# Asunatan/LM-Net

Measured on AMD Instinct MI355X. Metric: train images/sec at 352x352, 1/2/4/8 MI355X; Dice vs ref, higher is better.
Workload: dtype f32; 1 GPU; LM-Net fp32 training step (fwd + CE/Dice loss + bwd + AdamW), batch 8/GPU, 352x352 synthetic disc masks (BASELINE configs[1]); global_batch=8, parallelism=dp1, launch=lmn_plan_run (recorded C-side schedule, one crossing per pass)

## Files before the change

lm_net_amd/csrc/conv_common.h:

```cpp
#pragma once
#include "common.h"
#include <stdlib.h>

struct ConvParams {
  lmn_conv_args_t a;
  int nkb[3];
  int kb_off[3];
  int NKB;
  int NCTT;
  int ncls;
  int gpi;
  int ng_c[4];
  int Hc[4], Wc[4];
  int total_sets;
  float inv_keep_ep;
  float inv_keep_src[3];
  int TH, TW, TP, NG, XH, XW, CS, CKB, tiles_x, tiles_y, total_tiles;
  uint32_t mTW, mXW;
  int strided;
  float* det_stats;
  LmnLay lay_src[3], lay_out, lay_aux;
  int32_t rpw;
  uint32_t rp_magic;
  LmnLay lay_out2, lay_aux2;
  int32_t NCTT2;
  int32_t prio;
};

__device__ __forceinline__ void lmn_wave_prio(int mode) {
  uint32_t slot;
  asm volatile("s_getreg_b32 %0, hwreg(HW_REG_HW_ID, 0, 4)" : "=s"(slot));
  const uint32_t p = mode >= 4 ? (uint32_t)(7 - mode) : (mode == 2 ? 3u - (slot & 3u) : (mode == 3 ? (slot & 1u) * 3u : (slot & 3u)));
  switch (p) {
    case 0: __builtin_amdgcn_s_setprio(0); break;
    case 1: __builtin_amdgcn_s_setprio(1); break;
    case 2: __builtin_amdgcn_s_setprio(2); break;
    default: __builtin_amdgcn_s_setprio(3); break;
  }
}

__device__ __forceinline__ void lmn_wave_stagger(int units) {
  uint32_t slot;
  asm volatile("s_getreg_b32 %0, hwreg(HW_REG_HW_ID, 0, 4)" : "=s"(slot));
  const int n = (int)(slot & 7u) * units;
  for (int i = 0; i < n; ++i) __builtin_amdgcn_s_sleep(4);
}

namespace {

template <int PM> struct ActT { typedef float type; };
template <> struct ActT<2> { typedef lmn_bf16 type; };

typedef short s16x4 __attribute__((ext_vector_type(4)));
typedef __bf16 bf16x2_t __attribute__((ext_vector_type(2)));
typedef float f32x2_t __attribute__((ext_vector_type(2)));
__device__ __forceinline__ uint32_t pk_bf16(float a, float b) {
  const f32x2_t t = {a, b};
  return __builtin_bit_cast(uint32_t, __builtin_convertvector(t, bf16x2_t));
}
__device__ __forceinline__ uint2 pk4_bf16(f32x4 v) { return uint2{pk_bf16(v[0], v[1]), pk_bf16(v[2], v[3])}; }
template <bool BF> struct Frag { typedef f32x4 type; };
template <> struct Frag<true> { typedef uint2 type; };
template <bool BF> __device__ __forceinline__ typename Frag<BF>::type ldfrag(const float* p) {
  if constexpr (BF) return *reinterpret_cast<const uint2*>(p);
  else return *reinterpret_cast<const f32x4*>(p);
}
__device__ __forceinline__ f32x4 mfma_bf16(uint2 a, uint2 b, f32x4 c) {
  return __builtin_amdgcn_mfma_f32_16x16x16bf16_1k(__builtin_bit_cast(s16x4, a), __builtin_bit_cast(s16x4, b), c, 0, 0, 0);
}
typedef __bf16 bf16x8_t __attribute__((ext_vector_type(8)));
__device__ __forceinline__ f32x4 mfma_bf16x2(uint2 a0, uint2 a1, uint2 b0, uint2 b1, f32x4 c) {
#ifdef LMN_MFMA_X2
  const uint4 a = uint4{a0.x, a0.y, a1.x, a1.y}, b = uint4{b0.x, b0.y, b1.x, b1.y};
  return __builtin_amdgcn_mfma_f32_16x16x32_bf16(__builtin_bit_cast(bf16x8_t, a), __builtin_bit_cast(bf16x8_t, b), c, 0, 0, 0);
#else
  return mfma_bf16(a1, b1, mfma_bf16(a0, b0, c));
#endif
}

#ifdef LMN_CT_TIMING
__device__ unsigned long long g_ct_timing[4096 * 8];
#define LMN_TK(i) do { tk_b = __builtin_amdgcn_s_memtime(); tk_s[i] += tk_b - tk_a; tk_a = tk_b; } while (0)
#define LMN_TK_DRAIN() __builtin_amdgcn_s_waitcnt(0)
#else
#define LMN_TK(i) do { } while (0)
#define LMN_TK_DRAIN() do { } while (0)
#endif

}

int lmn_launch_conv_tile_1x1(const ConvParams& T, dim3 grid, size_t shmem, hipStream_t st, int tnct, int pm, int ek, bool rp, bool ln);
int lmn_launch_conv_tile_3x3(const ConvParams& T, dim3 grid, size_t shmem, hipStream_t st, int tnct, int pm, int ek, bool wlk, bool up);
int lmn_launch_conv_tile_3x3g(const ConvParams& T, dim3 grid, size_t shmem, hipStream_t st, int tnct, int pm, int ek, bool wlk);
size_t lmn_conv_dma3_lds(int C, int nct);
int lmn_launch_conv_dma3(const ConvParams& T, int blocks, hipStream_t st);
size_t lmn_conv_dmaM_lds(int XH, int XW);
bool lmn_conv_dmaM_fits(int XH, int XW);
int lmn_launch_conv_dmaM(const ConvParams& T, dim3 grid, hipStream_t st, int ek);
int lmn_conv_dma1_tp(int ks0, int ks1, int ks2, int aq, int nct, int mode, int gs, int nct2, int mode2);
size_t lmn_conv_dma1_lds(int ks0, int ks1, int ks2, int aq, int nct, int tp, int nct2);
int lmn_launch_conv_dma1(const ConvParams& T, int ks0, int ks1, int ks2, int aq, int nct, int mode, int gs, int nct2, int mode2, int blocks, hipStream_t st);
int lmn_launch_conv_tile_s2t(const ConvParams& T, dim3 grid, size_t shmem, hipStream_t st, int tnct, int pm, int ek);
int lmn_launch_conv_tileM(const ConvParams& T, dim3 grid, size_t shmem, hipStream_t st, int taps, int ncw, int pm, int ek, bool rp, bool ln, bool up);
```

lm_net_amd/csrc/conv_fwd.hip:

```cpp
#include "conv_common.h"

namespace {

struct PackGeom {
  int taps, Cout, Cin, nsrc, cs[3], transposed, row_off, rows;
  int bf16;
};

__device__ __forceinline__ float pack_element(const float* __restrict__ w, const PackGeom& g, int64_t i) {
  int nkb[3], kboff[3], cbase[3], NKB = 0, cb = 0;
#pragma unroll
  for (int s = 0; s < 3; ++s) {
    nkb[s] = s < g.nsrc ? (g.cs[s] + 15) / 16 : 0;
    kboff[s] = NKB;
    cbase[s] = cb;
    NKB += nkb[s];
    cb += s < g.nsrc ? g.cs[s] : 0;
  }
  const int nrows = g.transposed ? g.rows : g.Cout;
  const int NCTT = (nrows + 15) / 16;
  const int j = (int)(i & 3);
  const int lane = (int)((i >> 2) & 63);
  uint32_t t = (uint32_t)(i >> 8);
  const int ct = (int)(t % (uint32_t)NCTT);
// ... 148 lines not shown
  if (c < cinw) {
    const float zx = be[e] * m[c] + acc;
    dW[(int64_t)e * cinw + c] += a * R[(int64_t)e * rows + c] + b * zx + k * m[c];
  } else if (db) {
    const float zs = count * be[e] + acc;
    db[e] += a * hstats[e] + b * zs + k * count;
  }
}

}

thread_local char g_lmn_err[256] = {0};

extern "C" {

int lmn_abi_version(void) { return LMN_ABI_VERSION; }
int lmn_sizeof_conv_args(void) { return (int)sizeof(lmn_conv_args_t); }
int lmn_sizeof_src(void) { return (int)sizeof(lmn_src_t); }
int lmn_sizeof_pack_job(void) { return (int)sizeof(lmn_pack_job_t); }
const char* lmn_last_error(void) { return g_lmn_err; }
#ifdef LMN_CT_TIMING
int lmn_ct_timing(unsigned long long* out, int n) {
  return (int)hipMemcpyFromSymbol(out, HIP_SYMBOL(g_ct_timing), sizeof(unsigned long long) * n);
}
#endif

int64_t lmn_conv_pack_size(int ksize, int Cout, int nsrc, const int32_t* c) {
  int64_t nkb = 0;
  for (int s = 0; s < nsrc; ++s) nkb += (c[s] + 15) / 16;
  return (int64_t)ksize * ksize * nkb * ((Cout + 15) / 16) * 256;
}

int lmn_conv_pack(const float* w, float* wpack, int ksize, int Cout, int Cin, int nsrc, const int32_t* c,
                  int transposed, int row_off, int rows, int dtype, lmn_stream_t stream) {
  LMN_REQUIRE(w && wpack && c, "conv_pack: null pointer");
  LMN_REQUIRE(dtype == LMN_F32 || dtype == LMN_BF16, "conv_pack: dtype %d", dtype);
  if (g_lmn_rec && nsrc >= 1 && nsrc <= 3) {
    int32_t cc[3] = {c[0], nsrc > 1 ? c[1] : 0, nsrc > 2 ? c[2] : 0};
    const int32_t c0 = cc[0], c1 = cc[1], c2 = cc[2];
    lmn_rec_push([=]() -> int { const int32_t ca[3] = {c0, c1, c2}; return lmn_conv_pack(w, wpack, ksize, Cout, Cin, nsrc, ca, transposed, row_off, rows, dtype, stream); }, "lmn_conv_pack(");
  }
  LMN_REQUIRE(ksize == 1 || ksize == 3, "conv_pack: ksize %d", ksize);
  LMN_REQUIRE(nsrc >= 1 && nsrc <= 3, "conv_pack: nsrc %d", nsrc);
  int csum = 0;
  for (int s = 0; s < nsrc; ++s) csum += c[s];
  if (!transposed) {
    LMN_REQUIRE(csum == Cin || (nsrc == 1 && csum > Cin && csum < Cin + 4),
                "conv_pack: sources sum to %d channels, weight has %d", csum, Cin);
  } else {
    LMN_REQUIRE(nsrc == 1 && c[0] >= Cout && c[0] < Cout + 4, "conv_pack(transposed): one source of Cout=%d channels expected", Cout);
    LMN_REQUIRE(row_off >= 0 && rows > 0 && row_off + rows < Cin + 4, "conv_pack(transposed): rows [%d,+%d) of %d", row_off, rows, Cin);
  }
  const int nrows = transposed ? rows : (Cout + 3) / 4 * 4;
  const int64_t total = lmn_conv_pack_size(ksize, nrows, nsrc, c);
  LMN_REQUIRE(total < (1LL << 31), "conv_pack: %lld packed elements (32-bit index arithmetic)", (long long)total);
  const int blocks = (int)((total + 255) / 256 > 4096 ? 4096 : (total + 255) / 256);
  PackGeom g;
  g.taps = ksize * ksize; g.Cout = Cout; g.Cin = Cin; g.nsrc = nsrc;
  g.cs[0] = c[0]; g.cs[1] = nsrc > 1 ? c[1] : 0; g.cs[2] = nsrc > 2 ? c[2] : 0;
  g.transposed = transposed; g.row_off = row_off; g.rows = rows;
  g.bf16 = dtype == LMN_BF16;
  LMN_LAUNCH(conv_pack_kernel, dim3(blocks), dim3(256), 0, (hipStream_t)stream, w, wpack, g, total);
  return lmn_launch_status("conv_pack");
}

int lmn_conv_pack_batch(const lmn_pack_job_t* jobs_dev, int njobs, int64_t total_blocks, lmn_stream_t stream) {
  LMN_REC(lmn_conv_pack_batch(jobs_dev, njobs, total_blocks, stream));
  LMN_REQUIRE(jobs_dev && njobs > 0 && total_blocks > 0 && total_blocks < (1LL << 31), "conv_pack_batch: bad job table");
  LMN_LAUNCH(conv_pack_batch_kernel, dim3((unsigned)total_blocks), dim3(256), 0, (hipStream_t)stream, jobs_dev, njobs);
  return lmn_launch_status("conv_pack_batch");
}

static int g_conv_dma_mode = -1;
static int g_conv_dma_min_tiles = 512;
int lmn_conv_dma_config(int mode, int min_tiles) {
  const int prev = g_conv_dma_mode;
  if (mode >= 0) g_conv_dma_mode = mode;
  if (min_tiles >= 0) g_conv_dma_min_tiles = min_tiles;
  return prev;
}

struct Dma1Sel { int ks[3]; int aq, nct, mode, gs, nct2, mode2, tp; };
static bool dma1_select(const lmn_conv_args_t& A, Dma1Sel& S) {
  if (g_conv_dma_mode < 0) { const char* e = getenv("LMN_CONV_DMA"); g_conv_dma_mode = e ? atoi(e) : 7; }
  if (!(g_conv_dma_mode & 2)) return false;
  if (A.ksize != 1 || A.stride != 1 || A.mma_dtype != LMN_F32 || A.act_dtype != LMN_F32 || A.drop_p != 0.f || A.fin.mode != LMN_FIN_NONE || A.residual) return false;
  if (A.nsrc < 1 || A.nsrc > 3 || A.Cout <= 0 || A.Cout % 4 || A.Cout > 48 || A.out_rp_w < 0) return false;
  if (A.Hin != A.Hout || A.Win != A.Wout) return false;
  S.ks[0] = S.ks[1] = S.ks[2] = 0;
  S.gs = 0;
  for (int s = 0; s < A.nsrc; ++s) {
    const lmn_src_t& X = A.src[s];
    if (!X.ptr || X.C <= 0 || X.C % 4 || X.C > 48) return false;
    if (s == 0 && X.flags == LMN_SRC_GELU) S.gs = 1;
    else if (X.flags != 0 || X.scale) return false;
    if (X.rp_w && X.rp_w != A.Win) return false;
    S.ks[s] = X.C / 4;
  }
  if ((A.out_rp_w && A.out_rp_w != A.Win) || (A.aux && A.aux_rp_w && A.aux_rp_w != A.Win)) return false;
  const bool sebwd = A.epilogue == LMN_EP_SE_BWD && A.stats_mode == LMN_STATS_EP && A.aux && A.stats;
  S.mode = sebwd ? 5 : ((A.epilogue == LMN_EP_LINEAR && A.stats_mode == LMN_STATS_SUM_SQ && A.stats) ? 2 : ((A.epilogue == LMN_EP_LINEAR && A.stats_mode == LMN_STATS_NONE) ? 0 : -1));
  if (S.mode < 0 || (!sebwd && A.aux)) return false;
  S.nct = (A.Cout + 15) / 16;
  S.aq = sebwd ? A.Cout / 4 : 0;
  S.nct2 = S.mode2 = 0;
  int64_t maxc = A.Cout > A.out_cstride ? A.Cout : A.out_cstride;
  if (sebwd && A.aux_cstride > maxc) maxc = A.aux_cstride;
  for (int s = 0; s < A.nsrc; ++s) maxc = A.src[s].cstride > maxc ? A.src[s].cstride : maxc;
  const lmn_conv_chain_t& C2 = A.chain;
  if (C2.wpack) {
    if (S.mode != 0 || !A.out || !C2.out || C2.Cout <= 0 || C2.Cout % 4 || C2.Cout > 48 || g_lmn_det) return false;
    if ((C2.out_rp_w && C2.out_rp_w != A.Win) || (C2.aux && C2.aux_rp_w && C2.aux_rp_w != A.Win)) return false;
    const bool se2 = C2.epilogue == LMN_EP_SE_BWD && C2.stats_mode == LMN_STATS_EP && C2.aux && C2.stats;
    const bool sq2 = C2.epilogue == LMN_EP_LINEAR && C2.stats_mode == LMN_STATS_SUM_SQ && C2.stats && !C2.aux && C2.stats_rep >= 1;
    if (!se2 && !sq2) return false;
    S.mode2 = se2 ? 5 : 2;
    S.nct2 = (C2.Cout + 15) / 16;
    S.aq = se2 ? C2.Cout / 4 : 0;
    if (C2.Cout > maxc) maxc = C2.Cout;
    if (C2.out_cstride > maxc) maxc = C2.out_cstride;
    if (se2 && C2.aux_cstride > maxc) maxc = C2.aux_cstride;
  }
  S.tp = lmn_conv_dma1_tp(S.ks[0], S.ks[1], S.ks[2], S.aq, S.nct, S.mode, S.gs, S.nct2, S.mode2);
  if (S.tp <= 0) return false;
  const int64_t hw = (int64_t)A.Hin * A.Win, npx = (int64_t)A.B * hw;
  return hw % S.tp == 0 && npx / S.tp >= g_conv_dma_min_tiles && npx * maxc * 4 < 0x7fffffffLL;
}

int lmn_conv_chain_ok(const lmn_conv_args_t* args) {
  if (!args || !args->chain.wpack) return 0;
  Dma1Sel S;
  return dma1_select(*args, S) ? 1 : 0;
}

int lmn_conv_fwd(const lmn_conv_args_t* args, lmn_stream_t stream) {
  LMN_REQUIRE(args, "conv_fwd: null args");
  if (g_lmn_rec) {
    const lmn_conv_args_t copy = *args;
    lmn_rec_push([copy, stream]() -> int { return lmn_conv_fwd(&copy, stream); }, "lmn_conv_fwd(");
  }
  const lmn_conv_args_t& A = *args;
  if (A.chain.wpack) {
    Dma1Sel Sc;
    LMN_REQUIRE(dma1_select(A, Sc), "conv_fwd: these arguments do not take a chained second conv (lmn_conv_chain_ok says so beforehand)");
  }
  LMN_REQUIRE(A.ksize == 1 || A.ksize == 3, "conv_fwd: ksize %d", A.ksize);
  LMN_REQUIRE(A.stride == 1 || A.stride == 2, "conv_fwd: stride %d", A.stride);
  LMN_REQUIRE(A.nsrc >= 1 && A.nsrc <= 3, "conv_fwd: nsrc %d", A.nsrc);
  LMN_REQUIRE(A.Cout > 0 && A.Cout % 4 == 0, "conv_fwd: Cout %d must be a positive multiple of 4", A.Cout);
  LMN_REQUIRE(A.mma_dtype == LMN_F32 || A.mma_dtype == LMN_BF16, "conv_fwd: mma_dtype %d", A.mma_dtype);
  LMN_REQUIRE(A.act_dtype == LMN_F32 || (A.act_dtype == LMN_BF16 && A.mma_dtype == LMN_BF16),
              "conv_fwd: act_dtype %d with mma_dtype %d (bf16 storage needs bf16 matrix-core operands)", A.act_dtype, A.mma_dtype);
  LMN_REQUIRE(A.B > 0 && A.Hout > 0 && A.Wout > 0 && A.Hin > 0 && A.Win > 0, "conv_fwd: empty tensor");
  LMN_REQUIRE(A.wpack, "conv_fwd: null packed weights");
  LMN_REQUIRE(A.out || A.stats, "conv_fwd: neither out nor stats requested");
  LMN_REQUIRE(!(A.transposed && A.nsrc != 1), "conv_fwd: transposed form takes one source");
  {
    static int trace = -1;
    if (trace < 0) { const char* e = getenv("LMN_CONV_TRACE"); trace = e ? atoi(e) : 0; }
    if (trace) {
      fprintf(stderr, "conv_fwd k%d s%d T%d B%d %dx%d->%dx%d nsrc%d C", A.ksize, A.stride, A.transposed, A.B, A.Hin, A.Win, A.Hout, A.Wout, A.nsrc);
      for (int s = 0; s < A.nsrc; ++s) fprintf(stderr, "%s%d/%d(f%d%s%s)", s ? "+" : "", A.src[s].C, A.src[s].cstride, A.src[s].flags, A.src[s].scale ? "s" : "", A.src[s].rp_w ? "r" : "");
      fprintf(stderr, " Cout%d/%d ep%d st%d act%d drop%g res%d aux%d fin%d mma%d adt%d orp%d bias%d%d\n", A.Cout, A.out_cstride, A.epilogue, A.stats_mode, A.act, (double)A.drop_p,
              A.residual != nullptr, A.aux != nullptr, A.fin.mode, A.mma_dtype, A.act_dtype, A.out_rp_w, A.bias != nullptr, A.bias2 != nullptr);
    }
  }
  ConvParams P;
// ... 234 lines not shown
    int maxkb = 0;
    for (int s = 0; s < a.nsrc; ++s) maxkb = P.nkb[s] > maxkb ? P.nkb[s] : maxkb;
    T.CKB = maxkb < 2 ? maxkb : 2;
    if (ncw && a.ksize == 1) {
      static int ckb_cap = -1;
      if (ckb_cap < 0) { const char* e = getenv("LMN_CONVM_CKB"); ckb_cap = e ? atoi(e) : 8; }
      int c = maxkb < ckb_cap ? maxkb : ckb_cap;
      while (c > 2 && (size_t)T.TP * (c * 16 + 8) * sizeof(float) > 37 * 1024) --c;
      if (c > T.CKB) T.CKB = c;
    }
    if (ncw && a.ksize == 3 && !up2) {
      static int ckb3_env = -1;
      if (ckb3_env < 0) { const char* e = getenv("LMN_CONVM_CKB3"); ckb3_env = e ? atoi(e) : 8; }
      const long mblk = (long)a.B * ((gW + T.TW - 1) / T.TW) * ((gH + T.TH - 1) / T.TH) * ((P.NCTT + 4 * ncw - 1) / (4 * ncw));
      const size_t lds_cap = mblk <= 288 ? 144 * 1024 : (mblk <= 576 ? 72 * 1024 : 0);
      for (int c = 8; c > 2; c >>= 1) {
        if (c > ckb3_env || c > maxkb) continue;
        const bool bf0 = a.mma_dtype == LMN_BF16;
        const size_t need = ((size_t)T.XH * T.XW * (c * (bf0 ? 8 : 16) + (bf0 ? 4 : 8)) + (2 + 9) * 4 * ncw * 16) * sizeof(float);
        if (need <= lds_cap) { T.CKB = c; break; }
      }
    }
    T.CS = T.CKB * 16 + (st_in == 1 ? 8 : 4);
    const bool bf = a.mma_dtype == LMN_BF16;
    const int pm = bf ? (a.act_dtype == LMN_BF16 ? 2 : 1) : 0;
    if (bf) T.CS = T.CKB * 8 + 4;
    T.tiles_x = (gW + T.TW - 1) / T.TW;
    T.tiles_y = (gH + T.TH - 1) / T.TH;
    T.total_tiles = a.B * T.tiles_x * T.tiles_y;
    T.strided = a.epilogue == LMN_EP_SE_BWD ? 0 : 1;
    T.mTW = (uint32_t)((1ull << 32) / (uint32_t)T.TW + 1);
    T.mXW = (uint32_t)((1ull << 32) / (uint32_t)T.XW + 1);
    LMN_REQUIRE(T.XH * T.XW < 65536, "conv_fwd: window too large");
    size_t shmem = ((size_t)T.XH * T.XW * T.CS + (2 + 9) * tnct * 16) * sizeof(float);
    static int wl_kb = -1;
    if (wl_kb < 0) { const char* e = getenv("LMN_CONV_WL_KB"); wl_kb = e ? atoi(e) : 32; }
    const size_t wl_bytes = (size_t)9 * T.CKB * tnct * (a.mma_dtype == LMN_BF16 ? 128 : 256) * sizeof(float);
    const bool wlk = a.ksize == 3 && !s2t && shmem + wl_bytes <= (size_t)wl_kb * 1024;
    if (wlk) shmem += wl_bytes;
    LMN_REQUIRE(ncw || shmem <= 64 * 1024, "conv_fwd: LDS window %zu B", shmem);
    int blocks = T.total_tiles;
    int maxb = 1280 / tchunks > 256 ? 1280 / tchunks : 256;
    if (npg == 4) {
      int per_cu = (int)((160 * 1024) / (shmem + 512));
      per_cu = per_cu > 5 ? 5 : (per_cu < 1 ? 1 : per_cu);
      maxb = 256 * per_cu / tchunks > 256 ? 256 * per_cu / tchunks : 256;
    }
    if (s2t) maxb = 320 / tchunks > 64 ? 320 / tchunks : 64;
    {
      static int maxb_env = -1;
      if (maxb_env < 0) { const char* e = getenv("LMN_CONV_MAXB"); maxb_env = e ? atoi(e) : 0; }
      if (maxb_env > 0 && a.ksize == 3 && !s2t) maxb = maxb_env / tchunks > 1 ? maxb_env / tchunks : 1;
    }
    if (blocks > maxb) blocks = maxb;
    int ek = 1;
    if (a.epilogue <= LMN_EP_AFFINE_ACT && a.stats_mode == LMN_STATS_NONE) ek = 0;
    else if (a.drop_p > 0.f) ek = 1;
    else if (a.epilogue == LMN_EP_LINEAR && a.stats_mode == LMN_STATS_SUM_SQ) ek = 2;
    else if (a.epilogue == LMN_EP_BN_BWD1 && a.stats_mode == LMN_STATS_EP) ek = 3;
    else if (a.epilogue == LMN_EP_BN_BWD2 && a.stats_mode == LMN_STATS_NONE) ek = 4;
    else if (a.epilogue == LMN_EP_SE_BWD && a.stats_mode == LMN_STATS_EP) ek = 5;
    else if (a.epilogue == LMN_EP_LN_BWD) ek = 6;
    int det_ns = 0;
    int64_t det_sz = 0;
    auto det_prep = [&](int nbx) -> int {
      if (!g_lmn_det || !a.stats || a.stats_mode == LMN_STATS_NONE) return 0;
      const bool sebwd = a.epilogue == LMN_EP_SE_BWD;
      det_ns = sebwd ? nbx * 4 : nbx;
      det_sz = sebwd ? (int64_t)a.B * a.Cout : 2 * (int64_t)a.Cout;
      lmn_det_begin(st);
      T.det_stats = lmn_det_slots(st, (size_t)det_ns * det_sz);
      LMN_REQUIRE(T.det_stats, "conv_fwd: deterministic mode: no scratch for %d x %lld statistics slots", det_ns, (long long)det_sz);
      return 0;
    };
    auto det_finish = [&]() { if (T.det_stats) lmn_det_sum(st, T.det_stats, det_ns, det_sz, a.stats); };
    if (ncw) {
      LMN_REQUIRE(a.epilogue != LMN_EP_LN_BWD, "conv_fwd: LN_BWD is an N-split epilogue (Cout <= 48)");
      const int mchunks = (P.NCTT + 4 * ncw - 1) / (4 * ncw);
      int mblocks = T.total_tiles;
      const int mmax = 2048 / mchunks > 256 ? 2048 / mchunks : 256;
      if (mblocks > mmax) mblocks = mmax;
      const dim3 mgrid(mblocks, mchunks);
      {
        if (g_conv_dma_mode < 0) { const char* e = getenv("LMN_CONV_DMA"); g_conv_dma_mode = e ? atoi(e) : 7; }
        const lmn_src_t& s0 = a.src[0];
        const bool dm_ok = (g_conv_dma_mode & 4) && a.ksize == 3 && a.stride == 1 && !up2 && !ln && pm == 0 && a.nsrc == 1 && s0.flags == 0 && !s0.scale && s0.rp_w == 0 &&
                           s0.C % 4 == 0 && s0.cstride % 4 == 0 && a.epilogue == LMN_EP_LINEAR && (ek == 0 || ek == 2) && a.drop_p == 0.f && !a.aux && a.fin.mode == LMN_FIN_NONE &&
                           !a.out_rp_w && a.Hin == a.Hout && a.Win == a.Wout && lmn_conv_dmaM_fits(T.XH, T.XW) &&
                           (int64_t)a.B * a.Hin * a.Win * s0.cstride * 4 < 0x7fffffffLL && (int64_t)9 * P.NKB * P.NCTT * 1024 < 0x7fffffffLL;
        if (dm_ok) {
          const int dchunks = (P.NCTT + 3) / 4;
          int dblocks = T.total_tiles;
          const int dmax = 2048 / dchunks > 256 ? 2048 / dchunks : 256;
          if (dblocks > dmax) dblocks = dmax;
          if (int rc = det_prep(dblocks)) return rc;
          LMN_REQUIRE(lmn_launch_conv_dmaM(T, dim3(dblocks, dchunks), st, ek) == 0, "conv_fwd: no LDS-DMA M-split instance for epilogue %d", ek);
          det_finish();
          return lmn_launch_status("conv_fwd(dmaM)");
        }
      }
      if (int rc = det_prep(mblocks)) return rc;
      const size_t msh = ((size_t)T.XH * T.XW * T.CS + (2 + 9) * 4 * ncw * 16 + (ln ? 2 * T.XH * T.XW : 0)) * sizeof(float);
      lmn_launch_conv_tileM(T, mgrid, msh, st, a.ksize == 1 ? 1 : 9, ncw, pm, ek, a.ksize == 1 && T.rpw != 0, ln, up2);
      det_finish();
      return lmn_launch_status("conv_fwd(tileM)");
    }
    if (s2t) {
      const dim3 zgrid(blocks, tchunks, 4);
      if (int rc = det_prep(blocks * 4)) return rc;
      lmn_launch_conv_tile_s2t(T, zgrid, shmem, st, tnct, pm, ek);
      det_finish();
      return lmn_launch_status("conv_fwd(tile, stride-2 data gradient)");
    }
    {
      if (g_conv_dma_mode < 0) { const char* e = getenv("LMN_CONV_DMA"); g_conv_dma_mode = e ? atoi(e) : 7; }
      const int dma_env = g_conv_dma_mode & 1;
      const lmn_src_t& s0 = a.src[0];
      const int64_t dtiles = (int64_t)a.B * ((a.Wout + 15) / 16) * ((a.Hout + 7) / 8);
      const bool dma_ok = dma_env != 0 && a.ksize == 3 && a.stride == 1 && !up2 && !ln && pm == 0 && a.nsrc == 1 && s0.flags == 0 && !s0.scale && s0.rp_w == 0 &&
                          (s0.C == 12 || s0.C == 24) && P.NCTT <= 2 && a.epilogue == LMN_EP_LINEAR && (a.stats_mode == LMN_STATS_NONE || a.stats_mode == LMN_STATS_SUM_SQ) &&
                          a.drop_p == 0.f && !a.aux && a.fin.mode == LMN_FIN_NONE && !a.out_rp_w && a.Hin == a.Hout && a.Win == a.Wout && dtiles >= g_conv_dma_min_tiles && dtiles < (1 << 30) &&
                          (int64_t)a.B * a.Hin * a.Win * s0.cstride * 4 < 0x7fffffffLL && (int64_t)a.B * a.Hout * a.Wout * a.out_cstride * 4 < 0x7fffffffLL &&
                          (!a.residual || (int64_t)a.B * a.Hout * a.Wout * a.res_cstride < 0x7fffffffLL);
      if (dma_ok) {
        ConvParams D = T;
        D.tiles_x = (a.Wout + 15) / 16; D.tiles_y = (a.Hout + 7) / 8; D.total_tiles = (int)dtiles;
        const size_t lds = lmn_conv_dma3_lds(s0.C, P.NCTT);
        int bpc = (int)((160 * 1024) / (lds + 256));
        bpc = bpc > 4 ? 4 : (bpc < 1 ? 1 : bpc);
        static int bpc3_env = -1;
        if (bpc3_env < 0) { const char* e = getenv("LMN_DMA3_BPC"); bpc3_env = e ? atoi(e) : 0; }
        if (bpc3_env > 0 && bpc > bpc3_env) bpc = bpc3_env;
        int dblocks = 256 * bpc;
        if (dblocks > D.total_tiles) dblocks = D.total_tiles;
        if (int rc = det_prep(dblocks)) return rc;
        D.det_stats = T.det_stats;
        LMN_REQUIRE(lmn_launch_conv_dma3(D, dblocks, st) == 0, "conv_fwd: no LDS-DMA instance for C=%d, %d cout tiles", s0.C, P.NCTT);
        det_finish();
        return lmn_launch_status("conv_fwd(dma3)");
      }
    }
    if (a.ksize == 1) {
      Dma1Sel S1;
      if (dma1_select(A, S1)) {
        ConvParams D = T;
        D.total_tiles = (int)((int64_t)A.B * A.Hin * A.Win / S1.tp);
        D.NCTT2 = S1.nct2;
        D.lay_out2 = lmn_lay_make(A.chain.out_rp_w, A.chain.Cout > 0 ? A.chain.Cout : 4, A.chain.out_cstride);
        D.lay_aux2 = lmn_lay_make(A.chain.aux_rp_w, A.chain.Cout > 0 ? A.chain.Cout : 4, A.chain.aux_cstride);
        if (S1.nct2) {
          LMN_REQUIRE((!A.chain.out_rp_w || A.chain.out_rp_w == A.Win) && (!A.chain.aux_rp_w || A.chain.aux_rp_w == A.Win), "conv_fwd: row-planar tensors of the chained conv belong to images of the call's width");
          if (A.chain.out_rp_w || A.chain.aux_rp_w) { D.rpw = A.Win; D.rp_magic = lmn_div_magic(A.Win); }
        }
        const size_t lds = lmn_conv_dma1_lds(S1.ks[0], S1.ks[1], S1.ks[2], S1.aq, S1.nct, S1.tp, S1.nct2);
        int bpc = (int)((160 * 1024) / (lds + 256));
        bpc = bpc > 4 ? 4 : (bpc < 1 ? 1 : bpc);
        static int bpc1_env = -1;
        if (bpc1_env < 0) { const char* e = getenv("LMN_DMA1_BPC"); bpc1_env = e ? atoi(e) : 0; }
        if (bpc1_env > 0 && bpc > bpc1_env) bpc = bpc1_env;
        int dblocks = 256 * bpc;
        if (dblocks > D.total_tiles) dblocks = D.total_tiles;
        if (int rc = det_prep(dblocks)) return rc;
        D.det_stats = T.det_stats;
        LMN_REQUIRE(lmn_launch_conv_dma1(D, S1.ks[0], S1.ks[1], S1.ks[2], S1.aq, S1.nct, S1.mode, S1.gs, S1.nct2, S1.mode2, dblocks, st) == 0, "conv_fwd: LDS-DMA 1x1 instance table out of step");
        det_finish();
        return lmn_launch_status("conv_fwd(dma1)");
      }
    }
    const dim3 grid(blocks, tchunks);
    LMN_REQUIRE(a.epilogue != LMN_EP_LN_BWD || (tchunks == 1 && a.ksize == 1 && T.rpw == 0 && !ln), "conv_fwd: LN_BWD needs every cout in one block (N-split 1x1 NHWC call)");
    if (int rc = det_prep(blocks)) return rc;
    if (a.ksize == 1) lmn_launch_conv_tile_1x1(T, grid, shmem, st, tnct, pm, ek, T.rpw != 0, ln);
#ifdef LMN_CONV_NPG4
    else if (npg == 4) lmn_launch_conv_tile_3x3g(T, grid, shmem, st, tnct, pm, ek, wlk);
#endif
    else lmn_launch_conv_tile_3x3(T, grid, shmem, st, tnct, pm, ek, wlk, up2);
    det_finish();
    return lmn_launch_status("conv_fwd(tile)");
  }
  LMN_REQUIRE(false, "conv_fwd: the data gradient of a stride-2 conv is implemented for 3x3 kernels (got ksize %d, epilogue %d)", A.ksize, A.epilogue);
  return -1;
}

int lmn_reparam_fold(const float* hstats, const float* mean, const float* rstd, const float* A, float count, int batch_stats,
                     const float* w_expand, const float* b_expand, const float* w_shortcut, int E, int rows, int cin_w, int cred,
                     int cout_w, float* wpack, float* kbias, float* coef, float* dgamma, float* dbeta, int dtype,
                     lmn_stream_t stream) {
  LMN_REC(lmn_reparam_fold(hstats, mean, rstd, A, count, batch_stats, w_expand, b_expand, w_shortcut, E, rows, cin_w, cred, cout_w,
                           wpack, kbias, coef, dgamma, dbeta, dtype, stream));
  LMN_REQUIRE(hstats && mean && rstd && A && w_expand && b_expand && w_shortcut && wpack && kbias && coef && count > 0.f,
              "reparam_fold: null pointer");
  LMN_REQUIRE(E > 0 && rows > 0 && rows % 4 == 0 && cin_w > 0 && cin_w <= rows && cout_w > 0 && cout_w <= cred && cred % 4 == 0,
              "reparam_fold: E=%d rows=%d cin=%d cred=%d cout=%d", E, rows, cin_w, cred, cout_w);
  LMN_REQUIRE(dtype == LMN_F32 || dtype == LMN_BF16, "reparam_fold: dtype %d", dtype);
  FoldParams P;
  P.hstats = hstats; P.mean = mean; P.rstd = rstd; P.A = A; P.we = w_expand; P.be = b_expand; P.wsc = w_shortcut;
  P.wpack = wpack; P.kbias = kbias; P.coef = coef; P.dgamma = dgamma; P.dbeta = dbeta; P.count = count; P.batch_stats = batch_stats;
  P.E = E; P.rows = rows; P.cinw = cin_w; P.cred = cred; P.coutw = cout_w; P.bf16 = dtype == LMN_BF16;
// ... 30 lines not shown
```

lm_net_amd/csrc/conv_unity.hip:

```cpp
#include "conv_fwd.hip"
#include "conv_tile_1x1.hip"
#include "conv_tile_3x3.hip"
#include "conv_tileM.hip"
#include "conv_wgrad.hip"
#include "conv_dma3.hip"
#include "conv_dma1.hip"
#include "conv_dmaM.hip"
```

Before: 584.8 images/sec.

## Add LDS-DMA multi-stage pipelined kernel for wide 1x1 convolutions

Result: no change. 590.6 images/sec (median of 6 runs) (+1.0%).

```diff
diff --git a/lm_net_amd/csrc/conv_common.h b/lm_net_amd/csrc/conv_common.h
--- a/lm_net_amd/csrc/conv_common.h
+++ b/lm_net_amd/csrc/conv_common.h
@@ -97,6 +97,8 @@
 size_t lmn_conv_dmaM_lds(int XH, int XW);
 bool lmn_conv_dmaM_fits(int XH, int XW);
 int lmn_launch_conv_dmaM(const ConvParams& T, dim3 grid, hipStream_t st, int ek);
+size_t lmn_conv_dmaM1_lds(int ng, int ncw);
+int lmn_launch_conv_dmaM1(const ConvParams& T, dim3 grid, hipStream_t st, int ng, int ncw, int ek);
 int lmn_conv_dma1_tp(int ks0, int ks1, int ks2, int aq, int nct, int mode, int gs, int nct2, int mode2);
 size_t lmn_conv_dma1_lds(int ks0, int ks1, int ks2, int aq, int nct, int tp, int nct2);
 int lmn_launch_conv_dma1(const ConvParams& T, int ks0, int ks1, int ks2, int aq, int nct, int mode, int gs, int nct2, int mode2, int blocks, hipStream_t st);
diff --git a/lm_net_amd/csrc/conv_dmaM1.hip b/lm_net_amd/csrc/conv_dmaM1.hip
--- /dev/null
+++ b/lm_net_amd/csrc/conv_dmaM1.hip
@@ -0,0 +1,230 @@
+#include "conv_tile.h"
+
+namespace {
+
+constexpr unsigned M1_OOB = 0x80000000u;
+typedef int m1_i32x4 __attribute__((ext_vector_type(4)));
+__device__ __forceinline__ m1_i32x4 m1_rsrc(const void* p, unsigned bytes) {
+  const unsigned long long a = (unsigned long long)p;
+  m1_i32x4 r;
+  r.x = __builtin_amdgcn_readfirstlane((int)(unsigned)a);
+  r.y = __builtin_amdgcn_readfirstlane((int)(unsigned)(a >> 32));
+  r.z = __builtin_amdgcn_readfirstlane((int)bytes);
+  r.w = 0x00020000;
+  return r;
+}
+__device__ __forceinline__ void m1_piece(unsigned ldsaddr, unsigned voff, m1_i32x4 rsrc) {
+  unsigned keep;
+  asm volatile("s_mov_b32 %0, m0\n\ts_mov_b32 m0, %1\n\ts_nop 0\n\tbuffer_load_dwordx4 %2, %3, 0 offen lds\n\ts_mov_b32 m0, %0"
+               : "=&s"(keep) : "s"(ldsaddr), "v"(voff), "s"(rsrc) : "memory");
+}
+template <int N> __device__ __forceinline__ void m1_wait() { asm volatile("s_waitcnt vmcnt(%0)" ::"n"(N) : "memory"); }
+
+constexpr int M1_PS = 5;
+constexpr int m1_wp(int ng) { return (ng * 16 * M1_PS + 63) / 64; }
+constexpr int m1_npw(int ng, int ncw) { return (m1_wp(ng) + 4 * ncw + 3) / 4; }
+constexpr int m1_ring(int ng, int ncw) { return m1_wp(ng) + 4 * ncw <= 9 ? 4 : 3; }
+
+template <int NG, int NCW, int EPI>
+__global__ __launch_bounds__(256, 2) void conv_dmaM1_kernel(const ConvParams P) {
+  constexpr int TP = NG * 16, NCT = 4 * NCW;
+  constexpr int WP = m1_wp(NG), NPC = WP + NCT, NPW = m1_npw(NG, NCW), R = m1_ring(NG, NCW), D = R - 1;
+  constexpr int NCH = TP * M1_PS;
+  constexpr int SLOT = NPC * 256;
+  constexpr int NKP = (WP + 3) / 4;
+  static_assert((D - 1) * NPW <= 63, "vmcnt is a 6-bit counter");
+  const lmn_conv_args_t& A = P.a;
+  extern __shared__ __attribute__((aligned(16))) float smem[];
+  float* const s_dump = smem + R * SLOT;
+  float* const s_stats = s_dump + 256;
+  float* const s_par = s_stats + 2 * NCT * 16;
+  if (P.prio >= 4) lmn_setprio_level(7 - P.prio);
+  const int tid = threadIdx.x, lane = tid & 63;
+  const int wv = __builtin_amdgcn_readfirstlane(tid >> 6);
+  const int q = lane >> 4, n = lane & 15;
+  const int ct0 = blockIdx.y * NCT;
+  const int NPX = A.B * A.Win;
+  auto span = [&](int C, const LmnLay& L) -> unsigned {
+    const int64_t last = (int64_t)(NPX - 1) * L.cs + (int64_t)((C >> 2) - 1) * L.qs + 3 + (L.rf ? (int64_t)((NPX - 1) / P.rpw) * L.rf : 0);
+    return (unsigned)((last + 1) * 4);
+  };
+  const m1_i32x4 rs0 = m1_rsrc(A.src[0].ptr, span(A.src[0].C, P.lay_src[0]));
+  const m1_i32x4 rs1 = A.nsrc > 1 ? m1_rsrc(A.src[1].ptr, span(A.src[1].C, P.lay_src[1])) : rs0;
+  const m1_i32x4 rs2 = A.nsrc > 2 ? m1_rsrc(A.src[2].ptr, span(A.src[2].C, P.lay_src[2])) : rs0;
+  const m1_i32x4 rw = m1_rsrc(A.wpack, (unsigned)((int64_t)P.NKB * P.NCTT * 1024));
+  const unsigned lds0 = (unsigned)(size_t)(__attribute__((address_space(3))) void*)smem;
+  const unsigned dump0 = lds0 + (unsigned)(R * SLOT * 4);
+
+  int dpf[NKP];
+#pragma unroll
+  for (int k = 0; k < NKP; ++k) {
+    const int i = (k * 4 + wv) * 64 + lane;
+    const int px = i / M1_PS, f = i - px * M1_PS;
+    dpf[k] = (k * 4 + wv < WP && i < NCH && f < 4) ? (px << 8 | f) : -1;
+  }
+  int pgp[NKP], prow[NKP];
+  auto tile_addr = [&](int tile) __attribute__((always_inline)) {
+#pragma unroll
+    for (int k = 0; k < NKP; ++k) {
+      const int gp = tile * TP + (dpf[k] >> 8);
+      const bool ok = dpf[k] >= 0 && gp < NPX;
+      pgp[k] = ok ? gp : -1;
+      prow[k] = (ok && P.rpw) ? (int)lmn_div_row((uint32_t)gp, (uint32_t)P.rpw, P.rp_magic) : 0;
+    }
+  };
+  auto issue_stage = [&](int g) __attribute__((always_inline)) {
+    const unsigned sbase = lds0 + (unsigned)(g % R) * (unsigned)(SLOT * 4);
+    const bool real = g < P.NKB;
+    const int s = (A.nsrc > 2 && g >= P.kb_off[2]) ? 2 : ((A.nsrc > 1 && g >= P.kb_off[1]) ? 1 : 0);
+    const LmnLay L = P.lay_src[s];
+    const int qd0 = (g - P.kb_off[s]) * 4, CQ = A.src[s].C >> 2;
+#pragma unroll
+    for (int k = 0; k < NPW; ++k) {
+      const int p = k * 4 + wv;
+      if (k < NKP && p < WP) {
+        const int gp = pgp[k < NKP ? k : 0], qd = qd0 + (dpf[k < NKP ? k : 0] & 255);
+        const bool ok = real && gp >= 0 && qd < CQ;
+        const uint32_t off = (uint32_t)gp * (uint32_t)L.cs + (uint32_t)qd * (uint32_t)L.qs + (uint32_t)prow[k < NKP ? k : 0] * (uint32_t)L.rf;
+        const unsigned la = __builtin_amdgcn_readfirstlane(sbase + (unsigned)p * 1024u), vo = ok ? off * 4u : M1_OOB;
+        if (s == 2) m1_piece(la, vo, rs2); else if (s == 1) m1_piece(la, vo, rs1); else m1_piece(la, vo, rs0);
+      } else if (p < NPC) {
+        const int ct = min(ct0 + (p - WP), P.NCTT - 1);
+        m1_piece(__builtin_amdgcn_readfirstlane(sbase + (unsigned)p * 1024u), real ? (unsigned)((g * P.NCTT + ct) * 1024 + lane * 16) : M1_OOB, rw);
+      } else {
+        m1_piece(__builtin_amdgcn_readfirstlane(dump0), M1_OOB, rw);
+      }
+    }
+  };
+
+  for (int i = tid; i < 2 * NCT * 16; i += 256) s_stats[i] = 0.f;
+  conv_stage_params<NCT>(A, s_par, ct0, tid, blockIdx.x == 0);
+  float st0[NCW][4], st1[NCW][4];
+#pragma unroll
+  for (int c = 0; c < NCW; ++c)
+#pragma unroll
+    for (int r = 0; r < 4; ++r) st0[c][r] = st1[c][r] = 0.f;
+  __syncthreads();
+
+  const int nst = P.NKB;
+  for (int tile = blockIdx.x; tile < P.total_tiles; tile += gridDim.x) {
+    asm volatile("s_waitcnt vmcnt(0)" ::: "memory");
+    __builtin_amdgcn_s_barrier();
+    tile_addr(tile);
+#pragma unroll
+    for (int g = 0; g < D; ++g) issue_stage(g);
+    int opix[NG];
+    bool pvalid[NG];
+#pragma unroll
+    for (int g = 0; g < NG; ++g) {
+      const int gp = tile * TP + g * 16 + n;
+      pvalid[g] = gp < NPX;
+      opix[g] = pvalid[g] ? gp : 0;
+    }
+    f32x4 acc[NG][NCW];
+#pragma unroll
+    for (int c = 0; c < NCW; ++c) {
+      const f32x4 b4 = *reinterpret_cast<const f32x4*>(s_par + (wv + 4 * c) * 16 + q * 4);
+#pragma unroll
+      for (int g = 0; g < NG; ++g) acc[g][c] = b4;
+    }
+
+#pragma nounroll
+    for (int k = 0; k < nst; ++k) {
+      m1_wait<(D - 1) * NPW>();
+      __builtin_amdgcn_s_barrier();
+      issue_stage(k + D);
+      const float* XS = smem + (k % R) * SLOT;
+      const float* WS = XS + WP * 256 + n * 4 + q;
+      f32x4 xg[NG];
+      float w[NCW][4];
+#pragma unroll
+      for (int g = 0; g < NG; ++g) xg[g] = *reinterpret_cast<const f32x4*>(&XS[((g * 16 + n) * M1_PS + q) * 4]);
+#pragma unroll
+      for (int c = 0; c < NCW; ++c)
+#pragma unroll
+        for (int j = 0; j < 4; ++j) w[c][j] = WS[(wv + 4 * c) * 256 + j * 64];
+#pragma unroll
+      for (int j = 0; j < 4; ++j)
+#pragma unroll
+        for (int c = 0; c < NCW; ++c)
+#pragma unroll
+          for (int g = 0; g < NG; ++g) acc[g][c] = __builtin_amdgcn_mfma_f32_16x16x4f32(w[c][j], xg[g][j], acc[g][c], 0, 0, 0);
+    }
+
+#pragma unroll
+    for (int g = 0; g < NG; ++g) {
+      const uint32_t opx = (uint32_t)opix[g];
+      const uint32_t rowp = P.lay_out.rf ? lmn_div_row(opx, (uint32_t)P.rpw, P.rp_magic) : 0u;
+      const uint32_t oout = opx * (uint32_t)P.lay_out.cs + rowp * (uint32_t)P.lay_out.rf;
+#pragma unroll
+      for (int c = 0; c < NCW; ++c) {
+        const int ctc = ct0 + wv + 4 * c;
+        const int co = ctc * 16 + q * 4;
+        const bool cok = ctc < P.NCTT && co < A.Cout;
+        const bool live = pvalid[g] && cok;
+        const int cos = cok ? co : 0;
+        f32x4 o = acc[g][c];
+        if (EPI == 2 && live) {
+          const f32x4 sh = *reinterpret_cast<const f32x4*>(s_par + 6 * NCT * 16 + (wv + 4 * c) * 16 + q * 4);
+#pragma unroll
+          for (int r = 0; r < 4; ++r) { const float d = o[r] - sh[r]; st0[c][r] += d; st1[c][r] += d * d; }
+        }
+        if (A.residual) o += ld4((const float*)A.residual + opx * A.res_cstride + cos);
+        if (A.out && live) st4((float*)A.out + (oout + (uint32_t)(cos >> 2) * (uint32_t)P.lay_out.qs), o);
+      }
+    }
+  }
+
+  asm volatile("s_waitcnt vmcnt(0)" ::: "memory");
+
+  if (EPI == 2) {
+#pragma unroll
+    for (int c = 0; c < NCW; ++c)
+#pragma unroll
+      for (int r = 0; r < 4; ++r) {
+        float a = st0[c][r], bb = st1[c][r];
+#pragma unroll
+        for (int m = 1; m <= 8; m <<= 1) {
+          a += __shfl_xor(a, m, 64);
+          bb += __shfl_xor(bb, m, 64);
+        }
+        if (n == 0) {
+          s_stats[(wv + 4 * c) * 16 + q * 4 + r] = a;
+          s_stats[NCT * 16 + (wv + 4 * c) * 16 + q * 4 + r] = bb;
+        }
+      }
+    __syncthreads();
+    for (int i = tid; i < 2 * NCT * 16; i += 256) {
+      const int which = i / (NCT * 16), cc = i - which * NCT * 16;
+      const int co2 = ct0 * 16 + cc;
+      if (co2 < A.Cout) {
+        if (P.det_stats) P.det_stats[(int64_t)blockIdx.x * 2 * A.Cout + (int64_t)which * A.Cout + co2] = s_stats[i];
+        else atomicAdd(A.stats + (A.stats_rep > 1 ? (int64_t)(blockIdx.x % A.stats_rep) * 2 * A.Cout : 0) + (int64_t)which * A.Cout + co2, s_stats[i]);
+      }
+    }
+  }
+}
+
+}
+
+size_t lmn_conv_dmaM1_lds(int ng, int ncw) {
+  return ((size_t)m1_ring(ng, ncw) * (m1_wp(ng) + 4 * ncw) * 256 + 256 + (size_t)(2 + 9) * 4 * ncw * 16) * sizeof(float);
+}
+int lmn_launch_conv_dmaM1(const ConvParams& T, dim3 grid, hipStream_t st, int ng, int ncw, int ek) {
+  const size_t sh = lmn_conv_dmaM1_lds(ng, ncw);
+#define LMN_M1(GG, WW, EE)                                                                                                                  \
+  do {                                                                                                                                      \
+    if (sh > 64 * 1024) (void)hipFuncSetAttribute((const void*)conv_dmaM1_kernel<GG, WW, EE>, hipFuncAttributeMaxDynamicSharedMemorySize, (int)sh); \
+    LMN_LAUNCH((conv_dmaM1_kernel<GG, WW, EE>), grid, dim3(256), sh, st, T);                                                                \
+    return 0;                                                                                                                               \
+  } while (0)
+#define LMN_M1E(GG, WW) do { if (ek == 0) LMN_M1(GG, WW, 0); else LMN_M1(GG, WW, 2); } while (0)
+  if (ek != 0 && ek != 2) return -1;
+  if (ng == 2 && ncw == 1) LMN_M1E(2, 1);
+  if (ng == 2 && ncw == 2) LMN_M1E(2, 2);
+  if (ng == 4 && ncw == 1) LMN_M1E(4, 1);
+  if (ng == 4 && ncw == 2) LMN_M1E(4, 2);
+#undef LMN_M1E
+#undef LMN_M1
+  return -1;
+}
diff --git a/lm_net_amd/csrc/conv_fwd.hip b/lm_net_amd/csrc/conv_fwd.hip
--- a/lm_net_amd/csrc/conv_fwd.hip
+++ b/lm_net_amd/csrc/conv_fwd.hip
@@ -254,7 +254,7 @@
 
 struct Dma1Sel { int ks[3]; int aq, nct, mode, gs, nct2, mode2, tp; };
 static bool dma1_select(const lmn_conv_args_t& A, Dma1Sel& S) {
-  if (g_conv_dma_mode < 0) { const char* e = getenv("LMN_CONV_DMA"); g_conv_dma_mode = e ? atoi(e) : 7; }
+  if (g_conv_dma_mode < 0) { const char* e = getenv("LMN_CONV_DMA"); g_conv_dma_mode = e ? atoi(e) : 15; }
   if (!(g_conv_dma_mode & 2)) return false;
   if (A.ksize != 1 || A.stride != 1 || A.mma_dtype != LMN_F32 || A.act_dtype != LMN_F32 || A.drop_p != 0.f || A.fin.mode != LMN_FIN_NONE || A.residual) return false;
   if (A.nsrc < 1 || A.nsrc > 3 || A.Cout <= 0 || A.Cout % 4 || A.Cout > 48 || A.out_rp_w < 0) return false;
@@ -655,7 +655,7 @@
       if (mblocks > mmax) mblocks = mmax;
       const dim3 mgrid(mblocks, mchunks);
       {
-        if (g_conv_dma_mode < 0) { const char* e = getenv("LMN_CONV_DMA"); g_conv_dma_mode = e ? atoi(e) : 7; }
+        if (g_conv_dma_mode < 0) { const char* e = getenv("LMN_CONV_DMA"); g_conv_dma_mode = e ? atoi(e) : 15; }
         const lmn_src_t& s0 = a.src[0];
         const bool dm_ok = (g_conv_dma_mode & 4) && a.ksize == 3 && a.stride == 1 && !up2 && !ln && pm == 0 && a.nsrc == 1 && s0.flags == 0 && !s0.scale && s0.rp_w == 0 &&
                            s0.C % 4 == 0 && s0.cstride % 4 == 0 && a.epilogue == LMN_EP_LINEAR && (ek == 0 || ek == 2) && a.drop_p == 0.f && !a.aux && a.fin.mode == LMN_FIN_NONE &&
@@ -671,6 +671,49 @@
           det_finish();
           return lmn_launch_status("conv_fwd(dmaM)");
         }
+        bool m1_ok = (g_conv_dma_mode & 8) && a.ksize == 1 && a.stride == 1 && !up2 && !ln && pm == 0 && a.epilogue == LMN_EP_LINEAR && (ek == 0 || ek == 2) &&
+                     a.drop_p == 0.f && !a.aux && a.fin.mode == LMN_FIN_NONE && a.Win == a.Wout && ((uintptr_t)a.wpack & 15) == 0 &&
+                     (int64_t)P.NKB * P.NCTT * 1024 < 0x7fffffffLL;
+        const int64_t npx = (int64_t)a.B * a.Win;
+        for (int s = 0; m1_ok && s < a.nsrc; ++s) {
+          const lmn_src_t& x = a.src[s];
+          m1_ok = x.flags == 0 && !x.scale && x.C % 4 == 0 && x.cstride % 4 == 0 && ((uintptr_t)x.ptr & 15) == 0 && npx * x.cstride * 4 < 0x7fffffffLL;
+        }
+        if (m1_ok && a.out) m1_ok = a.out_cstride % 4 == 0 && ((uintptr_t)a.out & 15) == 0 && npx * a.out_cstride * 4 < 0x7fffffffLL;
+        if (m1_ok && a.residual) m1_ok = ((uintptr_t)a.residual & 15) == 0 && npx * a.res_cstride * 4 < 0x7fffffffLL;
+        {
+          static int m1_trace = -1;
+          if (m1_trace < 0) { const char* e = getenv("LMN_CONV_TRACE"); m1_trace = e ? atoi(e) : 0; }
+          if (m1_trace && a.ksize == 1) fprintf(stderr, "  conv_fwd wide 1x1: dmaM1 %s (ek %d, ln %d, pm %d)\n", m1_ok ? "takes it" : "rejects it", ek, (int)ln, pm);
+        }
+        if (m1_ok) {
+          static int m1_tp = -1, m1_ncw = -1;
+          if (m1_tp < 0) { const char* e = getenv("LMN_DMAM1_TP"); m1_tp = e ? atoi(e) : 0; }
+          if (m1_ncw < 0) { const char* e = getenv("LMN_DMAM1_NCW"); m1_ncw = e ? atoi(e) : 0; }
+          float mbest = 1e30f;
+          int bng = 4, bw = 1;
+          for (int ng = 4; ng >= 2; ng -= 2)
+            for (int w = 1; w <= 2; ++w) {
+              if ((m1_tp > 0 && m1_tp != ng * 16) || (m1_ncw > 0 && m1_ncw != w)) continue;
+              const int64_t blk = ((npx + ng * 16 - 1) / (ng * 16)) * ((P.NCTT + 4 * w - 1) / (4 * w));
+              const int bpc = (int)((160 * 1024) / (lmn_conv_dmaM1_lds(ng, w) + 512));
+              const float mf = (float)P.NKB * ng * w * 4 * 32, by = (float)P.NKB * (4 * w * 1024 + ng * 16 * 64) / 32.f;
+              const float cost = (float)((blk + 255) / 256) * (mf > by ? mf : by) + (float)((blk + 256 * bpc - 1) / (256 * bpc)) * (4000.f + 150.f * P.NKB);
+              if (cost < mbest * 0.999f) { mbest = cost; bng = ng; bw = w; }
+            }
+          ConvParams D = T;
+          D.TP = bng * 16; D.NG = bng;
+          D.total_tiles = (int)((npx + D.TP - 1) / D.TP);
+          const int dchunks = (P.NCTT + 4 * bw - 1) / (4 * bw);
+          int dblocks = D.total_tiles;
+          const int dmax = 2048 / dchunks > 256 ? 2048 / dchunks : 256;
+          if (dblocks > dmax) dblocks = dmax;
+          if (int rc = det_prep(dblocks)) return rc;
+          D.det_stats = T.det_stats;
+          LMN_REQUIRE(lmn_launch_conv_dmaM1(D, dim3(dblocks, dchunks), st, bng, bw, ek) == 0, "conv_fwd: no LDS-DMA 1x1 M-split instance for epilogue %d", ek);
+          det_finish();
+          return lmn_launch_status("conv_fwd(dmaM1)");
+        }
       }
       if (int rc = det_prep(mblocks)) return rc;
       const size_t msh = ((size_t)T.XH * T.XW * T.CS + (2 + 9) * 4 * ncw * 16 + (ln ? 2 * T.XH * T.XW : 0)) * sizeof(float);
@@ -686,7 +729,7 @@
       return lmn_launch_status("conv_fwd(tile, stride-2 data gradient)");
     }
     {
-      if (g_conv_dma_mode < 0) { const char* e = getenv("LMN_CONV_DMA"); g_conv_dma_mode = e ? atoi(e) : 7; }
+      if (g_conv_dma_mode < 0) { const char* e = getenv("LMN_CONV_DMA"); g_conv_dma_mode = e ? atoi(e) : 15; }
       const int dma_env = g_conv_dma_mode & 1;
       const lmn_src_t& s0 = a.src[0];
       const int64_t dtiles = (int64_t)a.B * ((a.Wout + 15) / 16) * ((a.Hout + 7) / 8);
diff --git a/lm_net_amd/csrc/conv_unity.hip b/lm_net_amd/csrc/conv_unity.hip
--- a/lm_net_amd/csrc/conv_unity.hip
+++ b/lm_net_amd/csrc/conv_unity.hip
@@ -6,3 +6,4 @@
 #include "conv_dma3.hip"
 #include "conv_dma1.hip"
 #include "conv_dmaM.hip"
+#include "conv_dmaM1.hip"
```
